# NVIDIA/cuopt

Hardware: AMD Instinct MI355X
Metric: pdlp_iterations_per_sec (higher is better)
Workload: dtype f64; 1 GPU; c3: synthetic random sparse LP S(m=1000000,n=1000000,k=10,seed=2), nnz=10000000, longest row 10, CSR fp64/int32, Stable2 preset, tolerances 0 (fixed iteration budget); rows=1000000, cols=1000000, nnz=10000000, parallelism=single GPU

## Files before the change

### cuopt_amd/capi.py

```python
import ctypes as C
import os

import numpy as np

_HERE = os.path.dirname(os.path.abspath(__file__))
LIB_PATH = os.environ.get("CUOPT_AMD_LIB") or os.path.join(_HERE, "lib", "libcuopt.so")

if not os.path.exists(LIB_PATH):
    raise ImportError(
        "cuopt_amd: %s is missing -- build it with `make -C cuopt_amd/csrc` (or "
        "`python -c 'import __graft_entry__ as g; g.build()'`). There is no CPU fallback." % LIB_PATH)

lib = C.CDLL(LIB_PATH, mode=C.RTLD_GLOBAL)

CUOPT_SUCCESS, CUOPT_INVALID_ARGUMENT, CUOPT_MPS_FILE_ERROR, CUOPT_MPS_PARSE_ERROR = 0, 1, 2, 3
CUOPT_VALIDATION_ERROR, CUOPT_OUT_OF_MEMORY, CUOPT_RUNTIME_ERROR = 4, 5, 6
CUOPT_MINIMIZE, CUOPT_MAXIMIZE = 1, -1
STATUS = {0: "NoTermination", 1: "Optimal", 2: "PrimalInfeasible", 3: "DualInfeasible",
          4: "IterationLimit", 5: "TimeLimit", 6: "NumericalError", 7: "PrimalFeasible",
          8: "FeasibleFound", 9: "ConcurrentLimit"}

c_int, c_double, c_void_p, c_char_p = C.c_int32, C.c_double, C.c_void_p, C.c_char_p
P = C.POINTER

# ... 254 lines not shown
if hasattr(lib, "pdlpdev_loop_stats"):
    _proto("pdlpdev_loop_stats", c_int, c_void_p, c_void_p)
    _proto("pdlpdev_run_period", c_int, c_void_p, c_int, c_void_p, c_void_p, c_void_p, c_void_p, c_void_p)
_proto("pdlpdev_save_best", c_int, c_void_p, c_int)
_proto("pdlpdev_trust_region_bounds", c_int, c_void_p, c_int, c_double, c_double, c_double, c_double, c_double, c_double, c_int, c_void_p)
_proto("pdlpdev_eval_infeasibility", c_int, c_void_p, c_int, c_int, c_void_p)
_proto("pdlpdev_get_solution", c_int, c_void_p, c_int, c_void_p, c_void_p, c_void_p)
_proto("pdlpdev_download", C.c_int64, c_void_p, c_int, c_void_p, C.c_int64)
_proto("pdlpdev_upload", C.c_int64, c_void_p, c_int, c_void_p, C.c_int64)
_proto("pdlpdev_spmv", c_int, c_void_p, c_int, c_void_p, c_void_p)
_proto("pdlpdev_time_kernel", c_int, c_void_p, c_int, c_int, P(c_double))
_proto("pdlpdev_synchronize", c_int, c_void_p)
_proto("pdlpdev_device_bytes", C.c_int64, c_void_p)
_proto("cuoptamd_dual_simplex", c_int, c_void_p, c_double, c_int, c_void_p, c_void_p, c_void_p, c_void_p, c_void_p, c_void_p, c_void_p)
_proto("cuoptamd_dual_simplex_from", c_int, c_void_p, c_void_p, c_void_p, c_double, c_int, c_void_p, c_void_p, c_void_p, c_void_p, c_void_p, c_void_p, c_void_p)
_proto("pdlpdev_shard_dataflow", c_int, c_void_p)
_proto("pdlpdev_shard_transport", c_int, c_void_p)
_proto("pdlpdev_shard_wire_bytes", c_int, c_void_p, c_void_p)
_proto("pdlpdev_dense_info", c_int, c_void_p, c_void_p)
_proto("pdlpdev_layout_info", c_int, c_void_p, c_void_p)
_proto("pdlpdev_comm_abort", c_int, c_void_p)
if hasattr(lib, "pdlpdev_shard_slice"):
    _proto("pdlpdev_shard_slice", c_int, c_void_p, P(c_int), P(c_int))
    _proto("pdlpdev_owner_layout_info", c_int, c_void_p, c_void_p)
_proto("pdlpdev_analyze", c_int, P(c_void_p), c_int, c_int, c_int, c_void_p, c_void_p, c_void_p, c_int)
_proto("pdlpdev_analysis_info", c_int, c_void_p, c_void_p)
_proto("pdlpdev_analysis_maps", c_int, c_void_p, c_void_p, c_void_p)
_proto("pdlpdev_analysis_download", c_int, c_void_p, c_int, c_void_p, c_void_p, c_void_p)
_proto("pdlpdev_create_from_analysis", c_int, P(c_void_p), c_void_p, c_void_p, c_void_p, c_void_p, c_void_p, c_void_p)
_proto("pdlpdev_analysis_destroy", None, c_void_p)
_proto("pdlpdev_debug_sort_pairs", c_int, c_int, C.c_int64, c_void_p, c_void_p, c_int, c_void_p, c_void_p)
_proto("pdlpdev_debug_scan", c_int, c_int, C.c_int64, c_void_p, c_void_p)
_proto("pdlpdev_debug_layout_checksums", c_int, c_void_p, c_void_p)
_proto("cuoptamd_solver_clone", c_int, c_void_p, c_void_p, c_void_p, c_void_p, c_void_p, c_void_p, P(c_void_p))
_proto("cuoptamd_batch_create", c_int, c_void_p, c_int, P(c_void_p))
_proto("cuoptamd_batch_advance", c_int, c_void_p, c_int, c_void_p)
_proto("cuoptamd_batch_destroy", None, c_void_p)
_proto("cuoptamd_batch_reset", c_int, c_void_p, c_void_p, c_void_p, c_void_p, c_void_p)
_proto("cuoptamd_batch_get_solutions", c_int, c_void_p, c_void_p, c_void_p, c_void_p)
_proto("cuoptamd_batch_branch", c_int, c_void_p, c_void_p, c_void_p, c_void_p)
_proto("cuoptamd_batch_solution_views", c_int, c_void_p, c_void_p, c_void_p, c_void_p)
_proto("cuoptamd_batch_device", c_void_p, c_void_p)
_proto("cuoptamd_batch_stats", c_int, c_void_p, c_void_p)
_proto("cuoptamd_batch_solve_last_path", C.c_char_p)
_proto("pdlpdev_small_batch_create", c_int, P(c_void_p), P(c_void_p), c_int)
_proto("pdlpdev_small_batch_destroy", None, c_void_p)
_proto("pdlpdev_create_share_stream", None, c_void_p)
_proto("pdlpdev_debug_ipc_export", c_int, c_int, c_int, c_void_p, P(c_void_p))
_proto("pdlpdev_debug_ipc_store", c_int, c_int, c_void_p, c_int, c_double)
_proto("pdlpdev_debug_ipc_wait", c_int, c_int, c_void_p, c_int, c_double)
_proto("pdlpdev_resident_size", c_int, c_int, c_int, C.c_int64)
if hasattr(lib, "pdlpdev_resident_tier"):
    _proto("pdlpdev_resident_tier", c_int, c_int, c_int, C.c_int64)
_proto("pdlpdev_batch_time_kernels", c_int, c_void_p, c_int, c_void_p)
_proto("pdlpdev_synthetic_lp", c_int, c_int, c_int, c_int, c_int, C.c_uint64, *([c_void_p] * 8))

if hasattr(lib, "pdlpdev_set_halpern"):
    _proto("pdlpdev_create_no_resident", None, c_int)
    _proto("pdlpdev_set_halpern", c_int, c_void_p, c_int)
    _proto("pdlpdev_spectral_norm", c_int, c_void_p, c_double, c_int, P(c_double), P(c_int))
    _proto("pdlpdev_halpern_restart", c_int, c_void_p, c_double, c_void_p, P(Ctl))
    _proto("pdlpdev_get_halpern", c_int, c_void_p, P(Halpern))
if hasattr(lib, "cuoptamd_solver_get_ray"):
    _proto("cuoptamd_solver_get_ray", c_int, c_void_p, c_void_p, c_void_p)
    _proto("pdlpdev_set_halpern_rays", c_int, c_void_p, c_int)
    _proto("pdlpdev_halpern_eval_infeasibility", c_int, c_void_p, c_int, c_void_p)
# ... 822 lines not shown
        def side(k):
            d = dict(layout=names[int(out[k])], panels=bool(out[k] == 1), workgroups=int(out[k + 1]))
            if out[k] == 3:
                d["lds_gather_saving_pct"] = int(out[k + 2])
            elif out[k] == 4:
                d["padding_pct"] = int(out[k + 2])
            else:
                d["slabs"] = int(out[k + 2])
                if out[k] == 1:
                    d["row_sums"] = "by_nonzero" if out[6 + k // 3] else "by_row"
            return d
        return dict(A=side(0), At=side(3), resident=bool(out[0] == 2))

    def shard_slice(self):
        a, b = c_int(), c_int()
        self._ck(lib.pdlpdev_shard_slice(self.handle, C.byref(a), C.byref(b)))
        return a.value, b.value

    def owner_layout(self):
        out = np.zeros(3, np.int32)
        self._ck(lib.pdlpdev_owner_layout_info(self.handle, _ptr(out)))
        return dict(layout={0: "stream", 1: "panel", 3: "jag", 4: "pb"}[int(out[0])], workgroups=int(out[1]), detail=int(out[2]))

    def wire_bytes(self):
        out = np.zeros(3, np.int64)
        self._ck(lib.pdlpdev_shard_wire_bytes(self.handle, _ptr(out)))
        return dict(halo=bool(out[0]), bytes=int(out[1]), bytes_allgather=int(out[2]))

    def layout_checksums(self):
        out = np.zeros(16, np.uint64)
        self._ck(lib.pdlpdev_debug_layout_checksums(self.handle, _ptr(out)))
        return out

    def dense_info(self):
        out = np.zeros(3, np.int64)
        self._ck(lib.pdlpdev_dense_info(self.handle, _ptr(out)))
        return dict(on=bool(out[0]), segments=int(out[1]), entries=int(out[2]))

    def time_kernel(self, kernel, reps=20):
        ms = c_double()
        self._ck(lib.pdlpdev_time_kernel(self.handle, KERNEL[kernel], int(reps), C.byref(ms)))
        return ms.value

    def close(self):
        if self.owner and self.handle:
            lib.pdlpdev_destroy(self.handle)
        self.handle = None

    def __del__(self):
        try:
            self.close()
        except Exception:
            pass
```

### cuopt_amd/csrc/kernels_layout_build.hip

```cpp
#include <hip/hip_runtime.h>

#include "pdlp_setup.hpp"
#include "setup_primitives.hpp"

namespace {

__global__ void __launch_bounds__(kT) k_panel_count(const int32_t* __restrict__ row0, const int32_t* __restrict__ off,
                                                    const int32_t* __restrict__ idx, int S, int32_t slab_w, int64_t own_from,
                                                    int32_t* __restrict__ count )
{
  __shared__ int c[16];
  if (threadIdx.x < 16) c[threadIdx.x] = 0;
  __syncthreads();
  const int w = blockIdx.x;
  const int32_t a = row0[w], b = row0[w + 1];
  for (int32_t i = a + threadIdx.x; i < b; i += kT) {
    const int32_t k0 = off[i], k1 = off[i + 1];
    if ((int64_t)(k1 - k0) > own_from) continue;
    int s_cur = -1, run = 0;
    for (int32_t k = k0; k < k1; ++k) {
      const int s2 = idx[k] / slab_w;
      if (s2 != s_cur) {
        if (run) atomicAdd(&c[s_cur], run);
        s_cur = s2, run = 0;
// ... 26 lines not shown
  }
  __syncthreads();
  for (int s2 = 0; s2 < S; ++s2) {
    int carry = 0;
    for (int r0 = 0; r0 < stride; r0 += 512) {
      const int r = r0 + threadIdx.x;
      const int v = r < nr ? (int)cnt[s2 * stride + r] : 0;
      int total   = 0;
      const int pre = block_exclusive_scan<512>(v, scratch, &total);
      if (r < stride) cnt[s2 * stride + r] = (unsigned short)(carry + pre);
      carry += total;
    }
  }
  __syncthreads();
  if (!SEG)
    for (int s2 = 0; s2 < S; ++s2) {
      uint16_t* dst = rowptr + rp_base[(size_t)w * S + s2];
      for (int r = threadIdx.x; r < stride; r += 512) dst[r] = cnt[s2 * stride + r];
    }
  __syncthreads();
  for (int32_t r = threadIdx.x; r < nr; r += 512) {
    const int32_t k0 = off[a + r], k1 = off[a + r + 1];
    if ((int64_t)(k1 - k0) > own_from) continue;
    for (int32_t k = k0; k < k1; ++k) {
      const int32_t c = idx[k];
      const int s2    = c / slab_w;
      const int32_t q = tile_ptr[(size_t)w * S + s2] + (int32_t)(cnt[s2 * stride + r]++);
      perm[q] = k;
      col[q]  = SEG ? (int32_t)(((uint32_t)r << kSegColBits) | (uint32_t)(c - s2 * slab_w)) : c;
    }
  }
}


}

int build_panels_device(pdlpdev_ctx* c, pdlpdev_ctx::Panels* dst, int32_t rows, int32_t cols, const int32_t* h_off,
                        const int32_t* d_off, const int32_t* d_idx, const double* d_val, int64_t slab_bytes, bool force)
{
  PanelHost h;
  std::vector<char> is_own;
  int64_t own_nnz = 0, own_from = 0;
  const bool timing = getenv("CUOPT_AMD_TIMING") != nullptr;
  auto t_last = std::chrono::steady_clock::now();
  auto plap = [&](const char* what) {
    if (!timing) return;
    const auto now = std::chrono::steady_clock::now();
    fprintf(stderr, "[cuopt_amd setup]     panels: %-18s %6.2f ms\n", what, 1e3 * std::chrono::duration<double>(now - t_last).count());
    t_last = now;
  };
  if (!panel_plan(&h, rows, cols, h_off, slab_bytes, force, nullptr, &is_own, &own_nnz, &own_from)) return 0;
  plap("plan");
  const int W = h.W, S = h.S;
  const int64_t nnz = h_off[rows];
  h.nnz = (size_t)(nnz - own_nnz), h.rowptr_size = h.seg ? 0 : (size_t)S * ((size_t)rows + W);
  int32_t *row0 = nullptr, *tile_ptr = nullptr, *col = nullptr, *count = nullptr;
  uint16_t* rowptr = nullptr;
  int64_t* rp_base = nullptr;
  TRY(upload_i32(c, &row0, h.row0.data(), h.row0.size()));
  TRY(dev_alloc(c, &count, (size_t)W * S + 1));
  k_panel_count<<<W, kT, 0, c->stream>>>(row0, d_off, d_idx, S, h.slab_w, own_from, count);
  std::vector<int32_t> hc((size_t)W * S);
  HIP_TRY(hipMemcpyAsync(hc.data(), count, hc.size() * sizeof(int32_t), hipMemcpyDeviceToHost, c->stream));
  HIP_TRY(hipStreamSynchronize(c->stream));
  plap("count");
  h.tile_ptr.resize((size_t)W * S + 1);
// ... 12 lines not shown
      for (int s2 = 0; s2 < S; ++s2) h.rp_base[(size_t)w * S + s2] = rp + (int64_t)s2 * (nr + 1);
    }
  TRY(upload_i32(c, &tile_ptr, h.tile_ptr.data(), h.tile_ptr.size()));
  {
    auto pad = [](size_t b) { return (b + 255) & ~(size_t)255; };
    const size_t b_col = pad((h.nnz + 8) * sizeof(int32_t)), b_rp = pad((h.rowptr_size + 8) * sizeof(uint16_t)), b_val = pad((h.nnz + 8) * sizeof(double));
    char* block = nullptr;
    HIP_TRY(hipMalloc((void**)&block, 2 * b_col + b_rp + b_val));
    c->allocs.push_back(block);
    c->bytes += (int64_t)(2 * b_col + b_rp + b_val);
    dst->val  = (double*)block;
    col       = (int32_t*)(block + b_val);
    dst->perm = (int32_t*)(block + b_val + b_col);
    rowptr    = (uint16_t*)(block + b_val + 2 * b_col);
  }
  TRY(dev_alloc(c, &rp_base, h.rp_base.size()));
  HIP_TRY(hipMemcpyAsync(rp_base, h.rp_base.data(), h.rp_base.size() * sizeof(int64_t), hipMemcpyHostToDevice, c->stream));
  plap("alloc");
  {
    const size_t lds = (size_t)S * (kPanelMaxRows + 1) * sizeof(unsigned short);
    static std::mutex mu;
    static std::vector<int> done;
    {
      std::lock_guard<std::mutex> lock(mu);
      if (std::find(done.begin(), done.end(), c->device) == done.end()) {
        HIP_TRY(hipFuncSetAttribute((const void*)k_panel_place<false>, hipFuncAttributeMaxDynamicSharedMemorySize, 16 * (kPanelMaxRows + 1) * 2));
        HIP_TRY(hipFuncSetAttribute((const void*)k_panel_place<true>, hipFuncAttributeMaxDynamicSharedMemorySize, 16 * (kPanelMaxRows + 1) * 2));
        done.push_back(c->device);
      }
    }
    if (h.seg) k_panel_place<true><<<W, 512, lds, c->stream>>>(row0, d_off, d_idx, S, h.slab_w, own_from, tile_ptr, rp_base, rowptr, dst->perm, col);
    else k_panel_place<false><<<W, 512, lds, c->stream>>>(row0, d_off, d_idx, S, h.slab_w, own_from, tile_ptr, rp_base, rowptr, dst->perm, col);
    HIP_TRY(hipGetLastError());
  }
  HIP_TRY(hipStreamSynchronize(c->stream));
  plap("place");
  dst->v = PanelView{h.W, h.S, h.any_long ? 1 : 0, row0, tile_ptr, rowptr, rp_base, col, dst->val};
  dst->v.seg = h.seg ? 1 : 0, dst->v.slab_w = h.slab_w;
  dst->nent  = (int64_t)h.nnz;
  if (!h.own_row.empty()) {
    int32_t *own_row = nullptr, *own_ptr = nullptr;
    TRY(upload_i32(c, &own_row, h.own_row.data(), h.own_row.size()));
    TRY(upload_i32(c, &own_ptr, h.own_ptr.data(), h.own_ptr.size()));
    HIP_TRY(hipStreamSynchronize(c->stream));
    dst->v.NP = h.W, dst->v.W = h.W + (int)h.own_row.size();
    dst->v.own_row = own_row, dst->v.own_ptr = own_ptr;
    dst->v.csr_off = d_off, dst->v.csr_idx = d_idx, dst->v.csr_val = d_val;
  }
  dst->on = true;
  return 0;
}

namespace {
constexpr int kPbBinT  = 1024;
constexpr int kPbSortN = 16384;
static_assert(kPbCap <= kPbSortN && kPbMaxRows <= 1024, "a bin's entries / rows fit the LDS sorts");

__global__ void __launch_bounds__(kT) k_max_row_len(int32_t rows, const int32_t* __restrict__ off, int* __restrict__ out)
{
  int best = 0;
  for (int64_t r = (int64_t)blockIdx.x * kT + threadIdx.x; r < rows; r += (int64_t)gridDim.x * kT) best = max(best, off[r + 1] - off[r]);
  for (int d = 1; d < 64; d <<= 1) best = max(best, __shfl_xor(best, d, 64));
  if ((threadIdx.x & 63) == 0 && best > 0) atomicMax(out, best);
}

constexpr int kPbItems = (kPbCap + kPbBinT - 1) / kPbBinT;
template <int MODE>
__global__ void __launch_bounds__(kPbBinT)
k_pb_bin(const int32_t* __restrict__ row0, const int32_t* __restrict__ off, const int32_t* __restrict__ idx, int panel_shift, int gshift, int S, int B,
         int32_t* __restrict__ bin_size, int* __restrict__ maxpad, uint16_t* __restrict__ cnt, const int32_t* __restrict__ pstart,
         const int32_t* __restrict__ bin_e0, int32_t* __restrict__ perm, uint16_t* __restrict__ lidx, int32_t* __restrict__ piece_dst,
// ... 1099 lines not shown
```

### cuopt_amd/csrc/kernels_panel.hip

```cpp
#include <hip/hip_runtime.h>

#include "pdlp_kernel_decls.hpp"
#include "pdlp_layouts.hpp"
#include "pdlp_setup.hpp"
#include "spmv_panel.hpp"

template <bool SEG>
__global__ void __launch_bounds__(kPanelThreads)
k_panel_a_dual(PanelView P, const pdlpdev_ctl* __restrict__ ctl, const double* __restrict__ xbar,
               double* __restrict__ y0, double* __restrict__ y1, const double* __restrict__ lo,
               const double* __restrict__ hi, double* __restrict__ sumy, double* __restrict__ part, double* __restrict__ ycopy,
               const p2pdev::Push* __restrict__ push)
{
  if (!loop_active(ctl)) return;
  DualEpilogue e = DualEpilogue::make(ctl, y0, y1, lo, hi, sumy, ycopy, push);
  const bool masked = !SEG && P.zmask != nullptr && (P.zforce != 0 || ctl->zskip != 0);
  if (masked && blockIdx.x == 0 && threadIdx.x == 0)
    __hip_atomic_fetch_add(const_cast<unsigned long long*>(P.zmask) + 2 * ((size_t)(P.zcols + 127) / 128), 1ull, __ATOMIC_RELAXED, __HIP_MEMORY_SCOPE_AGENT);
  panel_block_zs<SEG>(P, xbar, e, part, masked);
  if (push) p2pdev::count_exchange(push);
}

template <bool SEG>
__global__ void __launch_bounds__(kPanelThreads)
// ... 177 lines not shown
                const std::vector<int32_t>* dense_first_seg, std::vector<char>* is_own_out, int64_t* own_nnz_out, int64_t* own_from_out)
{
  PanelHost& P = *out;
  const int64_t nnz = rows > 0 ? off[rows] : 0;
  if (rows <= 0 || cols <= 0 || nnz <= 0) return false;
  if (!force && (int64_t)cols * 8 <= 2 * (int64_t)1048576) return false;
  int S = (int)(((int64_t)cols * 8 + slab_bytes - 1) / slab_bytes);
  S     = std::max(1, std::min(S, 16));
  const int32_t slab_w = (cols + S - 1) / S;
  const int64_t cap = std::max<int64_t>(2048, cuopt_amd::tune_int("panel_nnz", 60000));
  int64_t long_nnz = 0;
  int32_t max_len  = 0;
  {
    constexpr int kParts = 16;
    int64_t part_long[kParts] = {0};
    int32_t part_max[kParts]  = {0};
    cuopt_amd::parallel_tasks(kParts, [&](int t) {
      const int32_t a = (int32_t)((int64_t)rows * t / kParts), b = (int32_t)((int64_t)rows * (t + 1) / kParts);
      int64_t ln = 0;
      int32_t mx = 0;
      for (int32_t i = a; i < b; ++i) {
        const int32_t len = off[i + 1] - off[i];
        if (len > kLongRow) ln += len;
        mx = std::max(mx, len);
      }
      part_long[t] = ln, part_max[t] = mx;
    }, (int64_t)rows * 8);
    for (int t = 0; t < kParts; ++t) long_nnz += part_long[t], max_len = std::max(max_len, part_max[t]);
  }
  {
    const long long want = cuopt_amd::tune_int("panel_seg", -1);
    P.seg = want == 1 || (want != 0 && long_nnz * 50 > nnz);
    if (slab_w > (1 << kSegColBits)) P.seg = false;
  }
  const int64_t own_from = P.seg ? std::max<int64_t>(kPanelOwnRow, std::min<int64_t>(cap, (nnz + 511) / 512)) : kPanelOwnRow;
  std::vector<char>& is_own = *is_own_out;
  is_own.assign((size_t)rows, 0);
  int64_t own_nnz = 0;
  const bool any_own = max_len > own_from || dense_first_seg != nullptr;
  if (any_own)
    for (int32_t i = 0; i < rows; ++i)
      if (off[i + 1] - off[i] > own_from || (dense_first_seg && (*dense_first_seg)[i] >= 0))
        is_own[i] = 1, P.own_row.push_back(i), own_nnz += off[i + 1] - off[i];
  auto cut = [&](int64_t tgt) {
    P.row0.assign(1, 0);
    int32_t start = 0;
    if (!any_own) {
      while (start < rows) {
        const int32_t last = (int32_t)std::min<int64_t>(rows, (int64_t)start + kPanelMaxRows);
        const int64_t lim  = (int64_t)off[start] + tgt;
        int32_t end = (int32_t)(std::upper_bound(off + start, off + last + 1, lim, [](int64_t v, int32_t o) { return v < (int64_t)o; }) - off) - 1;
        if (end < last && off[end] == off[start]) ++end;
        end = std::max(end, start + 1);
        P.row0.push_back(end);
        start = end;
      }
      return;
    }
    while (start < rows) {
      int32_t end = start;
      int64_t cnt = 0;
      while (end < rows && end - start < kPanelMaxRows) {
        const int64_t len = is_own[end] ? 0 : off[end + 1] - off[end];
        if (cnt > 0 && cnt + len > tgt) break;
        cnt += len;
        ++end;
// ... 61 lines not shown
        if (is_own[i]) continue;
        for (int32_t t = off[i]; t < off[i + 1]; ++t) {
          const int s2    = idx[t] / slab_w;
          const int32_t q = cursor[s2]++;
          P.perm[q] = t, P.col[q] = (int32_t)(((uint32_t)(i - a) << kSegColBits) | (uint32_t)(idx[t] - s2 * slab_w));
        }
      }
    }, nnz);
    P.ok = true;
    return P;
  }
  P.rowptr.reset(P.rowptr_size);
  P.rp_base.resize((size_t)W * S);
  cuopt_amd::parallel_tasks(W, [&](int w) {
    const int32_t a = P.row0[w], b = P.row0[w + 1], nr = b - a;
    const int64_t rp = (int64_t)S * ((int64_t)a + w);
    std::vector<int32_t> cursor(S);
    for (int s2 = 0; s2 < S; ++s2) {
      cursor[s2]                    = P.tile_ptr[(size_t)w * S + s2];
      P.rp_base[(size_t)w * S + s2] = rp + (int64_t)s2 * (nr + 1);
    }
    for (int32_t i = a; i < b; ++i) {
      for (int s2 = 0; s2 < S; ++s2)
        P.rowptr[(size_t)(P.rp_base[(size_t)w * S + s2] + (i - a))] = (uint16_t)(cursor[s2] - P.tile_ptr[(size_t)w * S + s2]);
      if (is_own[i]) continue;
      for (int32_t t = off[i]; t < off[i + 1]; ++t) {
        const int s2 = idx[t] / slab_w;
        const int32_t q = cursor[s2]++;
        P.perm[q] = t, P.col[q] = idx[t];
      }
    }
    for (int s2 = 0; s2 < S; ++s2)
      P.rowptr[(size_t)(P.rp_base[(size_t)w * S + s2] + nr)] = (uint16_t)(cursor[s2] - P.tile_ptr[(size_t)w * S + s2]);
  }, nnz);
  P.ok = true;
  return P;
}

int upload_panels(pdlpdev_ctx* c, pdlpdev_ctx::Panels* dst, const PanelHost& h, const int32_t* d_off, const int32_t* d_idx,
                         const double* d_val)
{
  if (!h.ok) return 0;
  int32_t *row0 = nullptr, *tile_ptr = nullptr, *col = nullptr;
  uint16_t* rowptr = nullptr;
  int64_t* rp_base = nullptr;
  TRY(upload_i32(c, &row0, h.row0.data(), h.row0.size()));
  TRY(upload_i32(c, &tile_ptr, h.tile_ptr.data(), h.tile_ptr.size()));
  TRY(upload_i32(c, &col, h.col.get(), h.nnz));
  TRY(upload_i32(c, &dst->perm, h.perm.get(), h.nnz));
  TRY(dev_alloc(c, &rowptr, h.rowptr_size));
  HIP_TRY(hipMemcpyAsync(rowptr, h.rowptr.get(), h.rowptr_size * sizeof(uint16_t), hipMemcpyHostToDevice, c->stream));
  TRY(dev_alloc(c, &rp_base, h.rp_base.size()));
  HIP_TRY(hipMemcpyAsync(rp_base, h.rp_base.data(), h.rp_base.size() * sizeof(int64_t), hipMemcpyHostToDevice, c->stream));
  TRY(dev_alloc(c, &dst->val, h.nnz));
  HIP_TRY(hipStreamSynchronize(c->stream));
  dst->v  = PanelView{h.W, h.S, h.any_long ? 1 : 0, row0, tile_ptr, rowptr, rp_base, col, dst->val};
  dst->v.seg = h.seg ? 1 : 0, dst->v.slab_w = h.slab_w;
  dst->nent = (int64_t)h.nnz;
  if (!h.own_row.empty()) {
    int32_t *own_row = nullptr, *own_ptr = nullptr;
    TRY(upload_i32(c, &own_row, h.own_row.data(), h.own_row.size()));
    TRY(upload_i32(c, &own_ptr, h.own_ptr.data(), h.own_ptr.size()));
    HIP_TRY(hipStreamSynchronize(c->stream));
    dst->v.NP = h.W, dst->v.W = h.W + (int)h.own_row.size();
    dst->v.own_row = own_row, dst->v.own_ptr = own_ptr;
    dst->v.csr_off = d_off, dst->v.csr_idx = d_idx, dst->v.csr_val = d_val;
  }
  dst->on = true;
  return 0;
}

int pick_layout(pdlpdev_ctx* c, pdlpdev_ctx::MatrixSide* side, const double* vec, double* out)
{
  pdlpdev_ctx::Panels* pn = &side->pan;
  if (!pn->on) return 0;
  hipEvent_t e0, e1;
  HIP_TRY(hipEventCreate(&e0));
  HIP_TRY(hipEventCreate(&e1));
  float ms_stream = 1e30f, ms_panel = 1e30f;
  for (int round = 0; round < 2; ++round)
    for (int which = 0; which < 2; ++which) {
      for (int rep = 0; rep < 4; ++rep) {
        if (rep == 1) HIP_TRY(hipEventRecord(e0, c->stream));
        if (which == 0)
          k_spmv_plain<<<stream_grid(side->nb), kBlock, 0, c->stream>>>(side->nb, side->rb, side->hot.off, side->hot.idx, side->hot.val, vec, out, (const double*)nullptr);
        else
          (pn->v.seg ? k_panel_plain<true> : k_panel_plain<false>)<<<pn->v.W, kPanelThreads, 0, c->stream>>>(pn->v, vec, out);
      }
      HIP_TRY(hipEventRecord(e1, c->stream));
      HIP_TRY(hipEventSynchronize(e1));
// ... 15 lines not shown
```

### cuopt_amd/csrc/pdlp_device.hip

```cpp
#include "pdlp_ctx.hpp"
#include "pdlp_layouts.hpp"
#include "pdlp_setup.hpp"
#include "halpern_decision.hpp"


__global__ void __launch_bounds__(kBlock) k_fill(int64_t n, double* __restrict__ d, double v)
{
  for (int64_t i = blockIdx.x * (int64_t)kBlock + threadIdx.x; i < n; i += (int64_t)gridDim.x * kBlock)
    d[i] = v;
}
__global__ void __launch_bounds__(kBlock) k_scale_vectors(int n, int m, double* __restrict__ c,
                                                          double* __restrict__ lb,
                                                          double* __restrict__ ub,
                                                          const double* __restrict__ dc,
                                                          double* __restrict__ lo,
                                                          double* __restrict__ hi,
                                                          const double* __restrict__ dr)
{
  const int tot = n > m ? n : m;
  for (int i = blockIdx.x * kBlock + threadIdx.x; i < tot; i += gridDim.x * kBlock) {
    if (i < n) {
      c[i]  = c[i] * dc[i];
      lb[i] = lb[i] / dc[i];
      ub[i] = ub[i] / dc[i];
// ... 1583 lines not shown
  return 0;
}
int64_t pdlpdev_device_bytes(pdlpdev_ctx* ctx) { return ctx->bytes; }
int pdlpdev_shard_dataflow(pdlpdev_ctx* ctx) { return !ctx->comm ? 0 : ctx->owner ? 3 : ctx->rsag ? 2 : 1; }
int pdlpdev_shard_transport(pdlpdev_ctx* ctx) { return ctx->p2p.on ? 1 : 0; }
int pdlpdev_shard_wire_bytes(pdlpdev_ctx* ctx, int64_t out[3])
{
  out[0] = ctx->halo.on ? 1 : 0, out[1] = ctx->halo.on ? ctx->halo.bytes : ctx->halo.bytes_allgather, out[2] = ctx->halo.bytes_allgather;
  return 0;
}
int pdlpdev_dense_info(pdlpdev_ctx* ctx, int64_t out[3])
{
  out[0] = ctx->dense.on ? 1 : 0, out[1] = ctx->dense.nseg, out[2] = ctx->dense.nent;
  return 0;
}
int pdlpdev_layout_info(pdlpdev_ctx* ctx, int32_t out[8])
{
  ctx->A.info(out), ctx->At.info(out + 3);
  out[6] = ctx->A.pan.on && ctx->A.pan.v.seg, out[7] = ctx->At.pan.on && ctx->At.pan.v.seg;
  if (ctx->small_resident) out[0] = out[3] = 2;
  return 0;
}

static uint64_t checksum_device(pdlpdev_ctx* ctx, const void* dev, size_t bytes)
{
  if (!dev || bytes == 0) return 0;
  std::vector<unsigned char> h(bytes);
  if (hipMemcpy(h.data(), dev, bytes, hipMemcpyDeviceToHost) != hipSuccess) return ~0ull;
  uint64_t f = 1469598103934665603ull;
  for (unsigned char b : h) f = (f ^ b) * 1099511628211ull;
  (void)ctx;
  return f;
}
int pdlpdev_debug_layout_checksums(pdlpdev_ctx* ctx, uint64_t out[16])
{
  HIP_TRY(hipSetDevice(ctx->device));
  HIP_TRY(hipStreamSynchronize(ctx->stream));
  for (int i = 0; i < 16; ++i) out[i] = 0;
  const size_t nnz = (size_t)ctx->nnz;
  out[0] = checksum_device(ctx, ctx->At.full.off, ((size_t)ctx->n + 1) * 4);
  out[1] = checksum_device(ctx, ctx->At.full.idx, nnz * 4);
  out[2] = checksum_device(ctx, ctx->At.full.val, nnz * 8);
  auto panels = [&](const pdlpdev_ctx::Panels& P, int32_t rows, uint64_t* o) {
    if (!P.on) return;
    const int NP = P.v.NP ? P.v.NP : P.v.W;
    o[0] = checksum_device(ctx, P.v.row0, ((size_t)NP + 1) * 4);
    o[1] = checksum_device(ctx, P.v.tile_ptr, ((size_t)NP * P.v.S + 1) * 4);
    o[2] = P.v.seg ? 0 : checksum_device(ctx, P.v.rowptr, (size_t)P.v.S * ((size_t)rows + NP) * 2);
    o[3] = checksum_device(ctx, P.v.col, (size_t)P.nent * 4);
    o[4] = checksum_device(ctx, P.perm, (size_t)P.nent * 4);
  };
  panels(ctx->A.pan, ctx->m, out + 3);
  panels(ctx->At.pan, ctx->n, out + 8);
  auto gather_free = [&](const pdlpdev_ctx::Pb& P, int64_t side_nnz, uint64_t* o) {
    if (!P.on) return;
    const PbView& v = P.v;
    o[0] = checksum_device(ctx, P.perm, (size_t)P.np * 4);
    o[1] = checksum_device(ctx, v.lidx, (size_t)P.np * 2);
    o[2] = checksum_device(ctx, v.piece_dst, (size_t)(P.np >> v.gshift) * 4);
    o[4] = checksum_device(ctx, v.wg_e0, ((size_t)v.nwg + 1) * 4) ^ (checksum_device(ctx, v.wg_panel, (size_t)v.nwg * 4) * 3) ^
           (checksum_device(ctx, v.bin_row0, ((size_t)v.B + 1) * 4) * 5) ^ (checksum_device(ctx, v.bin_e0, ((size_t)v.B + 1) * 4) * 7) ^
           (uint64_t)v.S * 17 ^ (uint64_t)v.gshift * 19 ^ (uint64_t)v.panel_shift * 23 ^ (uint64_t)P.p_threads * 29 ^ (uint64_t)v.wide * 31;
    if (v.wide) {
      o[3] = checksum_device(ctx, v.rib, (size_t)P.np * 2) ^ (checksum_device(ctx, v.step_lv, (size_t)(P.np >> 10)) * 3) ^ (uint64_t)v.nser * 37;
      if (v.nser) {
        int32_t ser_nnz = 0;
// ... 35 lines not shown
```

### cuopt_amd/csrc/pdlp_kernels.hpp

```cpp
#pragma once
#include <hip/hip_runtime.h>
#include <stdint.h>


#include "cuopt_amd/pdlp_device.h"

namespace pdlp {

typedef double vec4d __attribute__((ext_vector_type(4)));
typedef int vec4i __attribute__((ext_vector_type(4)));

constexpr int kBlock    = 256;
constexpr int kNnzTile  = 2048;
constexpr int kNnzBlock = kNnzTile - 4;
constexpr int kLongRow  = 128;
constexpr int kMaxRowsPerBlock = 1024;

template <int XOR_MASK>
__device__ __forceinline__ double swizzle_xor(double v)
{
  static_assert(XOR_MASK >= 1 && XOR_MASK <= 16, "ds_swizzle works inside 32 lanes");
  constexpr int pattern = (XOR_MASK << 10) | 0x1F;
  int lo = __double2loint(v), hi = __double2hiint(v);
  lo = __builtin_amdgcn_ds_swizzle(lo, pattern);
// ... 97 lines not shown
constexpr int kPeriodGuard = 0x100;
__device__ __forceinline__ bool period_guard_skips(const pdlpdev_ctl* ctl, int& arg)
{
  const bool guarded = (arg & kPeriodGuard) != 0;
  arg &= ~kPeriodGuard;
  return guarded && !period_reached(ctl);
}

__device__ __forceinline__ int xcd_remap(int b, int nb)
{
  const int per = (nb + 7) >> 3;
  const int v   = (b & 7) * per + (b >> 3);
  return v;
}



constexpr int kPanelThreads = 512;
constexpr int kPanelChunk   = 4096;
constexpr int kPanelMaxRows = 3584;
constexpr int kPanelWaves   = kPanelThreads / 64;

struct PanelView {
  int W, S;
  int any_long;
  const int32_t* __restrict__ row0;
  const int32_t* __restrict__ tile_ptr;
  const uint16_t* __restrict__ rowptr;
  const int64_t* __restrict__ rp_base;
  const int32_t* __restrict__ col;
  const double* __restrict__ val;
  const double* __restrict__ dense_add = nullptr;
  int seg = 0, slab_w = 0;
  int NP = 0;
  const int32_t* __restrict__ own_row = nullptr;
  const int32_t* __restrict__ own_ptr = nullptr;
  const int32_t* __restrict__ csr_off = nullptr;
  const int32_t* __restrict__ csr_idx = nullptr;
  const double* __restrict__ csr_val  = nullptr;
  const int32_t* __restrict__ dn_own_seg   = nullptr;
  const int32_t* __restrict__ dn_pan_ptr   = nullptr;
  const int32_t* __restrict__ dn_pan_seg   = nullptr;
  const int32_t* __restrict__ dn_seg_row   = nullptr;
  const int32_t* __restrict__ dn_seg_c0    = nullptr;
  const int32_t* __restrict__ dn_seg_len   = nullptr;
  const int32_t* __restrict__ dn_seg_ptr   = nullptr;
  const double* __restrict__ dn_val        = nullptr;
  const unsigned long long* __restrict__ zmask = nullptr;
  int zcols = 0, zforce = 0;
};
constexpr int kZsQuads        = 1152;
constexpr int kPanelOwnRow = 4096;
constexpr int kPanelDenseSegs = 32;
constexpr long long kPanelNotMine = 0x7FF8C0DEC0DEC0DELL;

constexpr int kPanelPer     = kPanelChunk / kPanelThreads;
constexpr int kPanelRowsPer = (kPanelMaxRows + kPanelThreads - 1) / kPanelThreads;
constexpr int kSegColBits = 20;
constexpr unsigned kSegColMask = (1u << kSegColBits) - 1u;

constexpr int kJagMaxGroup = 256;
constexpr int kJagBatchRows = 16384;
#ifndef CUOPT_AMD_JAG_U
#define CUOPT_AMD_JAG_U 8
#endif
constexpr int kJagU        = CUOPT_AMD_JAG_U;
constexpr int jag_window(int waves) { return waves == 16 ? 16384 : 8192; }
constexpr size_t jag_lds_bytes(int waves) { return sizeof(double) * (size_t)(jag_window(waves) + waves * kJagMaxGroup); }
constexpr long long kJagNotMine = 0x7FF8C0DEC0DEC0DELL;

struct JagView {
  int rows, waves, ngroups, nblk, nlong;
  const int32_t* __restrict__ row0;
  const int32_t* __restrict__ tile_e;
  const int32_t* __restrict__ tile_sr;
  const uint32_t* __restrict__ sr;
  const uint16_t* __restrict__ slot;
  const double* __restrict__ val;
  const int32_t* __restrict__ win;
  const int32_t* __restrict__ set_ptr;
  const int32_t* __restrict__ set_col;
  const int32_t* __restrict__ lr_ptr;
  const int32_t* __restrict__ lr_row;
  const int32_t* __restrict__ off;
  const int32_t* __restrict__ idx;
  const double* __restrict__ csr_val;
  const double* __restrict__ dense_add = nullptr;
};


constexpr int kPbThreads = 512;
constexpr int kPbCap     = 9088;
// ... 166 lines not shown
```

### cuopt_amd/csrc/pdlp_layouts.hpp

```cpp
#pragma once
#include "pdlp_ctx.hpp"

struct PanelHost {
  bool ok = false, any_long = false;
  bool seg = false;
  int32_t slab_w = 0;
  int W = 0, S = 0;
  std::vector<int32_t> own_row, own_ptr;
  std::vector<int32_t> row0, tile_ptr;
  std::vector<int64_t> rp_base;
  cuopt_amd::PoolArray<int32_t> perm, col;
  cuopt_amd::PoolArray<uint16_t> rowptr;
  size_t nnz = 0, rowptr_size = 0;
};

constexpr int64_t kPanelWorkingSetBytes = 4 * (int64_t)1048576;

struct LayoutPolicy {
  enum Mode { kAuto, kStream, kPanel, kJag, kPb, kTimed } mode = kAuto;
  int64_t slab_bytes = 0;
  int64_t ws_limit   = 0;
  bool pb_device = true, jag_device = true;
  bool try_jag() const { return mode == kAuto || mode == kJag || mode == kTimed; }
  bool want_pb(int32_t cols) const { return mode == kPb || (mode == kAuto && (int64_t)cols * 8 > 16 * slab_bytes); }
};
int layout_policy(LayoutPolicy* p);

struct JagHost {
  bool ok = false;
  int rows = 0, waves = 8, ngroups = 0, nblk = 0;
  std::vector<int32_t> row0, tile_e, tile_sr, win, set_ptr, set_col, lr_ptr, lr_row;
  cuopt_amd::PoolArray<uint32_t> sr;
  cuopt_amd::PoolArray<uint16_t> slot;
  cuopt_amd::PoolArray<int32_t> perm;
  size_t nsr = 0, nent = 0;
  double saving = 0.0;
};

// ... 91 lines not shown
```

### cuopt_amd/csrc/spmv_panel.hpp

```cpp
#pragma once
#include <type_traits>

#include "pdlp_kernels.hpp"

namespace pdlp {

struct PanelChunk {
  int s, c0, c1, t0;
  bool valid;
};
template <int R>
__device__ __forceinline__ void panel_load(const PanelView& P, double (&va)[kPanelPer], int (&ja)[kPanelPer], int c0, int c1)
{
#pragma unroll
  for (int u = 0; u < R; ++u) {
    int k = c0 + threadIdx.x + u * kPanelThreads;
    if (u == R - 1) k = k < c1 ? k : c1 - 1;
    va[u] = __builtin_nontemporal_load(P.val + k);
    ja[u] = __builtin_nontemporal_load(P.col + k);
  }
}
template <int R>
__device__ __forceinline__ void panel_products(const double* __restrict__ vec, double* prod, const double (&va)[kPanelPer],
                                               const int (&ja)[kPanelPer], int len)
{
  double x[R];
#pragma unroll
  for (int u = 0; u < R; ++u) x[u] = vec[ja[u]];
#pragma unroll
  for (int u = 0; u < R; ++u) {
    const int i = threadIdx.x + u * kPanelThreads;
    if (u < R - 1 || i < len) prod[i] = va[u] * x[u];
  }
}
template <int R>
__device__ __forceinline__ void panel_products_zs(const double* __restrict__ vec, double* prod, const double (&va)[kPanelPer],
                                                  const int (&ja)[kPanelPer], int len, const unsigned* zbits, int zbase)
{
  unsigned w[R];
#pragma unroll
  for (int u = 0; u < R; ++u) {
    const int wi = (ja[u] >> 5) - zbase;
    w[u]         = wi < kZsQuads * 4 ? zbits[wi] : ~0u;
  }
  double x[R];
#pragma unroll
  for (int u = 0; u < R; ++u) {
    x[u] = 0.0;
    if ((w[u] >> (ja[u] & 31)) & 1u) x[u] = vec[ja[u]];
  }
#pragma unroll
  for (int u = 0; u < R; ++u) {
    const int i = threadIdx.x + u * kPanelThreads;
    if (u < R - 1 || i < len) prod[i] = va[u] * x[u];
  }
}
constexpr int kZsPer = (kZsQuads + kPanelThreads - 1) / kPanelThreads;
__device__ __forceinline__ int panel_zs_first_quad(const PanelView& P, int s) { return (int)(((long long)s * P.slab_w) >> 7); }
__device__ __forceinline__ void panel_zs_load(const PanelView& P, int s, uint4 (&st)[kZsPer])
{
  const long long c1 = (long long)(s + 1) * P.slab_w;
  const int last     = (int)(c1 < P.zcols ? c1 : P.zcols) - 1;
  const int q0       = panel_zs_first_quad(P, s);
  int nq             = (last >> 7) - q0 + 1;
  nq                 = nq < kZsQuads ? nq : kZsQuads;
  const uint4* __restrict__ src = reinterpret_cast<const uint4*>(P.zmask) + q0;
#pragma unroll
  for (int k = 0; k < kZsPer; ++k) {
    const int q = threadIdx.x + k * kPanelThreads;
    st[k]       = uint4{0u, 0u, 0u, 0u};
    if (q < nq) st[k] = src[q];
  }
}
__device__ __forceinline__ void panel_zs_store(uint4* zq, const uint4 (&st)[kZsPer])
{
#pragma unroll
  for (int k = 0; k < kZsPer; ++k) {
    const int q = threadIdx.x + k * kPanelThreads;
    if (q < kZsQuads) zq[q] = st[k];
  }
}
#define PANEL_DISPATCH(rounds, CALL) \
  switch (rounds) {                   \
    case 1: CALL(1); break;           \
    case 2: CALL(2); break;           \
    case 3: CALL(3); break;           \
    case 4: CALL(4); break;           \
// ... 246 lines not shown
    panel_own_row(P, vec, epi, partials, w, NP, prod);
    return;
  }
  __shared__ PanelDenseSegs dseg;
  const int r0 = P.row0[w], nr = P.row0[w + 1] - r0;
  panel_dense_prepare(P, w, vec, &dseg);
  if (threadIdx.x <= P.S) tile_s[threadIdx.x] = P.tile_ptr[w * P.S + threadIdx.x];
  if (threadIdx.x < P.S) base_s[threadIdx.x] = P.rp_base[w * P.S + threadIdx.x];
  for (int r = threadIdx.x; r < nr; r += kPanelThreads) psum[r] = 0.0;
  __syncthreads();
  if (P.own_ptr)
    for (int q = P.own_ptr[w] + (int)threadIdx.x; q < P.own_ptr[w + 1]; q += kPanelThreads) psum[P.own_row[q] - r0] = __longlong_as_double(kPanelNotMine);
  auto advance = [&](PanelChunk c) -> PanelChunk {
    if (c.valid && c.c1 < tile_s[c.s + 1]) {
      c.c0 = c.c1;
      c.c1 = c.c0 + kPanelChunk < tile_s[c.s + 1] ? c.c0 + kPanelChunk : tile_s[c.s + 1];
      return c;
    }
    int s = c.s + 1;
    while (s < P.S && tile_s[s + 1] == tile_s[s]) ++s;
    c.valid = s < P.S;
    c.s     = s;
    if (c.valid) {
      c.t0 = c.c0 = tile_s[s];
      c.c1 = c.c0 + kPanelChunk < tile_s[s + 1] ? c.c0 + kPanelChunk : tile_s[s + 1];
    }
    return c;
  };
  double va[kPanelPer];
  int ja[kPanelPer];
  unsigned ext_next[kPanelRowsPer], ext[kPanelRowsPer];
#define PANEL_ROUNDS(c) (((c).c1 - (c).c0 + kPanelThreads - 1) / kPanelThreads)
#define PANEL_CALL_LOAD(R) panel_load<R>(P, va, ja, nxt.c0, nxt.c1)
#define PANEL_CALL_PRODUCTS(R) panel_products<R>(vec, prod, va, ja, cur.c1 - cur.c0)
#define PANEL_CALL_PRODUCTS_ZS(R) panel_products_zs<R>(vec, prod, va, ja, cur.c1 - cur.c0, reinterpret_cast<const unsigned*>(zq), panel_zs_first_quad(P, cur.s) << 2)
#define PANEL_REQUEST(c)                                                         \
  if ((c).valid) {                                                               \
    PANEL_DISPATCH(PANEL_ROUNDS(c), PANEL_CALL_LOAD)                             \
    const uint16_t* __restrict__ rp_ = P.rowptr + base_s[(c).s];                 \
    _Pragma("unroll") for (int q = 0; q < kPanelRowsPer; ++q) {                  \
      int r_      = threadIdx.x + q * kPanelThreads;                             \
      r_          = r_ < nr ? r_ : 0;                                            \
      ext_next[q] = (unsigned)rp_[r_] | ((unsigned)rp_[r_ + 1] << 16);           \
    }                                                                            \
  }
  PanelChunk none{-1, 0, 0, 0, false};
  PanelChunk nxt = advance(none);
  PANEL_REQUEST(nxt)
  PanelChunk cur = nxt;
  if (zon && cur.valid) {
    uint4 st[kZsPer];
    panel_zs_load(P, cur.s, st);
    panel_zs_store(zq, st);
  }
  constexpr bool kEarly = PanelEarlyOps<Epi>::on;
  [[maybe_unused]] typename PanelEarlyOps<Epi>::type pre[kPanelEpiDepth];
  [[maybe_unused]] int lo_last = 0, hi_last = 0;
  while (cur.valid) {
    __syncthreads();
    if (zon) { PANEL_DISPATCH(PANEL_ROUNDS(cur), PANEL_CALL_PRODUCTS_ZS) }
    else { PANEL_DISPATCH(PANEL_ROUNDS(cur), PANEL_CALL_PRODUCTS) }
#pragma unroll
    for (int q = 0; q < kPanelRowsPer; ++q) ext[q] = ext_next[q];
    const int lo = cur.c0 - cur.t0, hi = cur.c1 - cur.t0;
    nxt = advance(cur);
    if constexpr (kEarly)
      if (!nxt.valid) {
        lo_last = lo, hi_last = hi;
// ... 235 lines not shown
```

### include/cuopt_amd/pdlp_device.h

```cpp
#ifndef CUOPT_AMD_PDLP_DEVICE_H
#define CUOPT_AMD_PDLP_DEVICE_H

#include <stdint.h>

#ifdef __cplusplus
extern "C" {
#endif

typedef struct pdlpdev_ctx pdlpdev_ctx;

typedef struct pdlpdev_ctl {
  double step_size;
  double primal_weight;
  double tau;
  double sigma;
  double sum_weights;
  double last_interaction, last_movement, last_dx2, last_dy2;
  int32_t k;
  int32_t cur;
  int32_t pending_avg;
  int32_t steps_taken;
  int32_t attempts;
  int32_t target_steps;
  int32_t error;
// ... 94 lines not shown
void pdlpdev_create_no_resident(int no_resident);
void pdlpdev_create_batch_lanes(int lanes);
void pdlpdev_create_share_stream(pdlpdev_ctx* donor);
int pdlpdev_resident_size(int32_t m, int32_t n, int64_t nnz);
int pdlpdev_resident_tier(int32_t m, int32_t n, int64_t nnz);
int pdlpdev_create_overlapped(pdlpdev_ctx** out, int device, int32_t m, int32_t n, const int32_t* a_offsets,
                              const int32_t* a_indices, const double* a_values, const int32_t* at_offsets,
                              const int32_t* at_indices, const double* at_values,
                              void (*transpose_ready)(void*), void* user, const double* c, const double* lo,
                              const double* hi, const double* lb, const double* ub);
void pdlpdev_destroy(pdlpdev_ctx* ctx);

typedef struct pdlpdev_analysis pdlpdev_analysis;
int pdlpdev_analyze(pdlpdev_analysis** out, int device, int32_t m, int32_t n, const int32_t* a_offsets, const int32_t* a_indices,
                    const double* a_values, int flags);
int pdlpdev_analyze_with_vectors(pdlpdev_analysis** out, int device, int32_t m, int32_t n, const int32_t* a_offsets, const int32_t* a_indices,
                                 const double* a_values, int flags, const double* c, const double* lo, const double* hi, const double* lb,
                                 const double* ub);
int pdlpdev_analysis_info(pdlpdev_analysis* an, int32_t out[10]);
int pdlpdev_analysis_maps(pdlpdev_analysis* an, int32_t* row_new2old, int32_t* col_new2old);
int pdlpdev_analysis_vectors_in_order(pdlpdev_analysis* an);
void pdlpdev_analysis_release_workspace(pdlpdev_analysis* an);
int pdlpdev_analysis_download(pdlpdev_analysis* an, int which, int32_t* offsets, int32_t* indices, double* values);
int pdlpdev_create_from_analysis(pdlpdev_ctx** out, pdlpdev_analysis* an, const double* c, const double* lo, const double* hi,
                                 const double* lb, const double* ub);
void pdlpdev_analysis_destroy(pdlpdev_analysis* an);
int pdlpdev_debug_sort_pairs(int device, int64_t n, const uint32_t* keys, const uint32_t* vals, int bits, uint32_t* keys_out,
                             uint32_t* vals_out);
int pdlpdev_debug_scan(int device, int64_t n, const int32_t* in, int32_t* out);
int pdlpdev_debug_ipc_export(int device, int count, uint8_t handle[64], void** base);
int pdlpdev_debug_ipc_store(int device, const uint8_t handle[64], int count, double seed);
int pdlpdev_debug_ipc_wait(int device, void* base, int count, double seed);
int pdlpdev_debug_layout_checksums(pdlpdev_ctx* ctx, uint64_t out[16]);
int pdlpdev_debug_pb_wide_host(int32_t rows, int32_t cols, const int32_t* off, const int32_t* idx, const double* val, const double* x, double* out,
                               int64_t info[5]);
int pdlpdev_synthetic_lp(int device, int32_t m, int32_t n, int32_t k, uint64_t seed, int32_t* offsets, int32_t* indices, double* values,
                         double* c, double* lo, double* hi, double* x_star, double* y_star);

int pdlpdev_comm_unique_id(uint8_t id[128]);
int pdlpdev_comm_init(pdlpdev_ctx* ctx, int rank, int world, const uint8_t id[128]);

int pdlpdev_softcomm_create(int world, uint8_t id[128]);
int pdlpdev_comm_abort(const uint8_t id[128]);

int pdlpdev_scaling_compute(pdlpdev_ctx* ctx, int do_ruiz, int ruiz_iterations,
                            int do_pock_chambolle, double alpha);
int pdlpdev_scale_problem(pdlpdev_ctx* ctx);
int pdlpdev_init_norms(pdlpdev_ctx* ctx, double out[3]);
int pdlpdev_agree_max(pdlpdev_ctx* ctx, double* value);
int pdlpdev_weight_norms(pdlpdev_ctx* ctx, int unscaled, double out[2]);
int pdlpdev_reset(pdlpdev_ctx* ctx, const double* lb, const double* ub, const double* lo, const double* hi);
int pdlpdev_problem_norms(pdlpdev_ctx* ctx, double* norm_c, double* norm_b);
int pdlpdev_set_step_params(pdlpdev_ctx* ctx, const pdlpdev_step_params* p);
int pdlpdev_set_step(pdlpdev_ctx* ctx, double step_size, double primal_weight);
int pdlpdev_set_k(pdlpdev_ctx* ctx, int32_t k);
int pdlpdev_set_initial(pdlpdev_ctx* ctx, const double* x, const double* y);
int pdlpdev_project_primal(pdlpdev_ctx* ctx);
int pdlpdev_initial_solution_stats(pdlpdev_ctx* ctx, double out[5], const double* x0_unscaled, const double* y0_unscaled);

int pdlpdev_compute_aty(pdlpdev_ctx* ctx);
int pdlpdev_run(pdlpdev_ctx* ctx, int32_t target_steps, pdlpdev_ctl* ctl);
int pdlpdev_get_ctl(pdlpdev_ctx* ctx, pdlpdev_ctl* ctl);
typedef struct pdlpdev_batch pdlpdev_batch;
int pdlpdev_clone_shared(pdlpdev_ctx** out, pdlpdev_ctx* parent);
int pdlpdev_batch_create(pdlpdev_batch** out, pdlpdev_ctx** ctx, int K);
int pdlpdev_batch_run(pdlpdev_batch* batch, const int32_t* targets, pdlpdev_ctl* ctl);
// ... 85 lines not shown
```

Baseline: 6570 iterations/s.

## Sort panel chunk entries by column to improve gather locality in SpMV

Within each panel tile chunk, entries are reordered by column (on host and via a device bitonic sort kernel), with each column word packing the original slot index in its high bits. The SpMV product step decodes the column and scatters the product back to its original LDS slot, so x-vector gathers become more coalesced/cache-friendly. This costs extra decode ALU work, a scattered LDS write, and setup-time sorting; it is enabled by default for non-segmented panels.

New measurement: 6773 iterations/s (median of 6 runs). 3.1% higher.

```diff
diff --git a/cuopt_amd/capi.py b/cuopt_amd/capi.py
--- a/cuopt_amd/capi.py
+++ b/cuopt_amd/capi.py
@@ -310,6 +310,8 @@
 _proto("pdlpdev_debug_sort_pairs", c_int, c_int, C.c_int64, c_void_p, c_void_p, c_int, c_void_p, c_void_p)
 _proto("pdlpdev_debug_scan", c_int, c_int, C.c_int64, c_void_p, c_void_p)
 _proto("pdlpdev_debug_layout_checksums", c_int, c_void_p, c_void_p)
+if hasattr(lib, "pdlpdev_debug_panel_words"):
+    _proto("pdlpdev_debug_panel_words", c_int, c_void_p, c_int, c_void_p, c_void_p, c_void_p)
 _proto("cuoptamd_solver_clone", c_int, c_void_p, c_void_p, c_void_p, c_void_p, c_void_p, c_void_p, P(c_void_p))
 _proto("cuoptamd_batch_create", c_int, c_void_p, c_int, P(c_void_p))
 _proto("cuoptamd_batch_advance", c_int, c_void_p, c_int, c_void_p)
@@ -1198,6 +1200,13 @@
         self._ck(lib.pdlpdev_debug_layout_checksums(self.handle, _ptr(out)))
         return out
 
+    def panel_words(self, side):
+        which, info = dict(A=0, At=1)[side], np.zeros(5, np.int64)
+        self._ck(lib.pdlpdev_debug_panel_words(self.handle, which, _ptr(info), None, None))
+        tile_ptr, col = np.zeros(int(info[0] * info[1]) + 1, np.int32), np.zeros(int(info[2]), np.int32)
+        self._ck(lib.pdlpdev_debug_panel_words(self.handle, which, _ptr(info), _ptr(tile_ptr), _ptr(col)))
+        return dict(panels=int(info[0]), slabs=int(info[1]), sorted=bool(info[3]), slab_w=int(info[4]), tile_ptr=tile_ptr, col=col)
+
     def dense_info(self):
         out = np.zeros(3, np.int64)
         self._ck(lib.pdlpdev_dense_info(self.handle, _ptr(out)))
diff --git a/cuopt_amd/csrc/kernels_layout_build.hip b/cuopt_amd/csrc/kernels_layout_build.hip
--- a/cuopt_amd/csrc/kernels_layout_build.hip
+++ b/cuopt_amd/csrc/kernels_layout_build.hip
@@ -82,6 +82,38 @@
   }
 }
 
+__global__ void __launch_bounds__(512) k_panel_sort(int S, int32_t slab_w, const int32_t* __restrict__ tile_ptr, int32_t* __restrict__ perm,
+                                                    int32_t* __restrict__ col)
+{
+  __shared__ uint32_t key[kPanelChunk];
+  __shared__ int32_t pm[kPanelChunk];
+  const int32_t t1 = tile_ptr[blockIdx.x + 1], base = (int32_t)(blockIdx.x % (unsigned)S) * slab_w;
+  for (int32_t c0 = tile_ptr[blockIdx.x]; c0 < t1; c0 += kPanelChunk) {
+    const int len = t1 - c0 < kPanelChunk ? t1 - c0 : kPanelChunk;
+    int n = 2;
+    while (n < len) n <<= 1;
+    for (int i = threadIdx.x; i < n; i += 512) {
+      key[i] = i < len ? ((uint32_t)(col[c0 + i] - base) << 12) | (uint32_t)i : 0xFFFFFFFFu;
+      if (i < len) pm[i] = perm[c0 + i];
+    }
+    __syncthreads();
+    for (int k = 2; k <= n; k <<= 1)
+      for (int j = k >> 1; j > 0; j >>= 1) {
+        for (int t = threadIdx.x; t < (n >> 1); t += 512) {
+          const int lo = ((t & ~(j - 1)) << 1) | (t & (j - 1)), hi = lo | j;
+          const uint32_t a = key[lo], b = key[hi];
+          if ((a > b) == ((lo & k) == 0)) key[lo] = b, key[hi] = a;
+        }
+        __syncthreads();
+      }
+    for (int i = threadIdx.x; i < len; i += 512) {
+      const uint32_t slot = key[i] & 0xFFFu;
+      col[c0 + i]  = (int32_t)((slot << kSegColBits) | (key[i] >> 12));
+      perm[c0 + i] = pm[slot];
+    }
+    __syncthreads();
+  }
+}
 
 }
 
@@ -160,11 +192,15 @@
     if (h.seg) k_panel_place<true><<<W, 512, lds, c->stream>>>(row0, d_off, d_idx, S, h.slab_w, own_from, tile_ptr, rp_base, rowptr, dst->perm, col);
     else k_panel_place<false><<<W, 512, lds, c->stream>>>(row0, d_off, d_idx, S, h.slab_w, own_from, tile_ptr, rp_base, rowptr, dst->perm, col);
     HIP_TRY(hipGetLastError());
+    if (h.sorted) {
+      k_panel_sort<<<W * S, 512, 0, c->stream>>>(S, h.slab_w, tile_ptr, dst->perm, col);
+      HIP_TRY(hipGetLastError());
+    }
   }
   HIP_TRY(hipStreamSynchronize(c->stream));
   plap("place");
   dst->v = PanelView{h.W, h.S, h.any_long ? 1 : 0, row0, tile_ptr, rowptr, rp_base, col, dst->val};
-  dst->v.seg = h.seg ? 1 : 0, dst->v.slab_w = h.slab_w;
+  dst->v.seg = h.seg ? 1 : 0, dst->v.slab_w = h.slab_w, dst->v.sorted = h.sorted ? 1 : 0;
   dst->nent  = (int64_t)h.nnz;
   if (!h.own_row.empty()) {
     int32_t *own_row = nullptr, *own_ptr = nullptr;
diff --git a/cuopt_amd/csrc/kernels_panel.hip b/cuopt_amd/csrc/kernels_panel.hip
--- a/cuopt_amd/csrc/kernels_panel.hip
+++ b/cuopt_amd/csrc/kernels_panel.hip
@@ -233,6 +233,7 @@
     const long long want = cuopt_amd::tune_int("panel_seg", -1);
     P.seg = want == 1 || (want != 0 && long_nnz * 50 > nnz);
     if (slab_w > (1 << kSegColBits)) P.seg = false;
+    P.sorted = !P.seg && slab_w <= (1 << kSegColBits) && cuopt_amd::tune_int("panel_sort", 1) != 0;
   }
   const int64_t own_from = P.seg ? std::max<int64_t>(kPanelOwnRow, std::min<int64_t>(cap, (nnz + 511) / 512)) : kPanelOwnRow;
   std::vector<char>& is_own = *is_own_out;
@@ -360,6 +361,20 @@
     }
     for (int s2 = 0; s2 < S; ++s2)
       P.rowptr[(size_t)(P.rp_base[(size_t)w * S + s2] + nr)] = (uint16_t)(cursor[s2] - P.tile_ptr[(size_t)w * S + s2]);
+    if (!P.sorted) return;
+    std::vector<uint32_t> key;
+    std::vector<int32_t> pm;
+    for (int s2 = 0; s2 < S; ++s2)
+      for (int32_t c0 = P.tile_ptr[(size_t)w * S + s2], t1 = P.tile_ptr[(size_t)w * S + s2 + 1]; c0 < t1; c0 += kPanelChunk) {
+        const int32_t len = std::min<int32_t>(kPanelChunk, t1 - c0);
+        key.resize((size_t)len), pm.assign(&P.perm[c0], &P.perm[c0] + len);
+        for (int32_t i = 0; i < len; ++i) key[i] = ((uint32_t)(P.col[c0 + i] - s2 * slab_w) << 12) | (uint32_t)i;
+        std::sort(key.begin(), key.end());
+        for (int32_t i = 0; i < len; ++i) {
+          const uint32_t slot = key[i] & 0xFFFu;
+          P.col[c0 + i] = (int32_t)((slot << kSegColBits) | (key[i] >> 12)), P.perm[c0 + i] = pm[slot];
+        }
+      }
   }, nnz);
   P.ok = true;
   return P;
@@ -383,7 +398,7 @@
   TRY(dev_alloc(c, &dst->val, h.nnz));
   HIP_TRY(hipStreamSynchronize(c->stream));
   dst->v  = PanelView{h.W, h.S, h.any_long ? 1 : 0, row0, tile_ptr, rowptr, rp_base, col, dst->val};
-  dst->v.seg = h.seg ? 1 : 0, dst->v.slab_w = h.slab_w;
+  dst->v.seg = h.seg ? 1 : 0, dst->v.slab_w = h.slab_w, dst->v.sorted = h.sorted ? 1 : 0;
   dst->nent = (int64_t)h.nnz;
   if (!h.own_row.empty()) {
     int32_t *own_row = nullptr, *own_ptr = nullptr;
diff --git a/cuopt_amd/csrc/pdlp_device.hip b/cuopt_amd/csrc/pdlp_device.hip
--- a/cuopt_amd/csrc/pdlp_device.hip
+++ b/cuopt_amd/csrc/pdlp_device.hip
@@ -1639,6 +1639,18 @@
   (void)ctx;
   return f;
 }
+int pdlpdev_debug_panel_words(pdlpdev_ctx* ctx, int side, int64_t info[5], int32_t* tile_ptr, int32_t* col)
+{
+  HIP_TRY(hipSetDevice(ctx->device));
+  HIP_TRY(hipStreamSynchronize(ctx->stream));
+  const pdlpdev_ctx::Panels& P = side ? ctx->At.pan : ctx->A.pan;
+  if (!P.on) return fail(-1, "side %d is not in panels", side);
+  const int NP = P.v.NP ? P.v.NP : P.v.W;
+  info[0] = NP, info[1] = P.v.S, info[2] = P.nent, info[3] = P.v.sorted, info[4] = P.v.slab_w;
+  if (tile_ptr) HIP_TRY(hipMemcpy(tile_ptr, P.v.tile_ptr, ((size_t)NP * P.v.S + 1) * 4, hipMemcpyDeviceToHost));
+  if (col) HIP_TRY(hipMemcpy(col, P.v.col, (size_t)P.nent * 4, hipMemcpyDeviceToHost));
+  return 0;
+}
 int pdlpdev_debug_layout_checksums(pdlpdev_ctx* ctx, uint64_t out[16])
 {
   HIP_TRY(hipSetDevice(ctx->device));
diff --git a/cuopt_amd/csrc/pdlp_kernels.hpp b/cuopt_amd/csrc/pdlp_kernels.hpp
--- a/cuopt_amd/csrc/pdlp_kernels.hpp
+++ b/cuopt_amd/csrc/pdlp_kernels.hpp
@@ -153,6 +153,7 @@
   const double* __restrict__ val;
   const double* __restrict__ dense_add = nullptr;
   int seg = 0, slab_w = 0;
+  int sorted = 0;
   int NP = 0;
   const int32_t* __restrict__ own_row = nullptr;
   const int32_t* __restrict__ own_ptr = nullptr;
@@ -179,6 +180,7 @@
 constexpr int kPanelRowsPer = (kPanelMaxRows + kPanelThreads - 1) / kPanelThreads;
 constexpr int kSegColBits = 20;
 constexpr unsigned kSegColMask = (1u << kSegColBits) - 1u;
+static_assert(kPanelChunk <= 1 << 12, "a sorted chunk's slot takes the 12 bits beside the column");
 
 constexpr int kJagMaxGroup = 256;
 constexpr int kJagBatchRows = 16384;
diff --git a/cuopt_amd/csrc/pdlp_layouts.hpp b/cuopt_amd/csrc/pdlp_layouts.hpp
--- a/cuopt_amd/csrc/pdlp_layouts.hpp
+++ b/cuopt_amd/csrc/pdlp_layouts.hpp
@@ -4,6 +4,7 @@
 struct PanelHost {
   bool ok = false, any_long = false;
   bool seg = false;
+  bool sorted = false;
   int32_t slab_w = 0;
   int W = 0, S = 0;
   std::vector<int32_t> own_row, own_ptr;
diff --git a/cuopt_amd/csrc/spmv_panel.hpp b/cuopt_amd/csrc/spmv_panel.hpp
--- a/cuopt_amd/csrc/spmv_panel.hpp
+++ b/cuopt_amd/csrc/spmv_panel.hpp
@@ -20,39 +20,52 @@
     ja[u] = __builtin_nontemporal_load(P.col + k);
   }
 }
+__device__ __forceinline__ void panel_decode(int word, int i, bool sorted, int slab_base, int& col, int& slot)
+{
+  col  = sorted ? slab_base + (int)((unsigned)word & kSegColMask) : word;
+  slot = sorted ? (int)((unsigned)word >> kSegColBits) : i;
+}
 template <int R>
 __device__ __forceinline__ void panel_products(const double* __restrict__ vec, double* prod, const double (&va)[kPanelPer],
-                                               const int (&ja)[kPanelPer], int len)
+                                               const int (&ja)[kPanelPer], int len, bool sorted, int slab_base)
 {
   double x[R];
-#pragma unroll
-  for (int u = 0; u < R; ++u) x[u] = vec[ja[u]];
+  int slot[R];
+#pragma unroll
+  for (int u = 0; u < R; ++u) {
+    int c;
+    panel_decode(ja[u], threadIdx.x + u * kPanelThreads, sorted, slab_base, c, slot[u]);
+    x[u] = vec[c];
+  }
 #pragma unroll
   for (int u = 0; u < R; ++u) {
     const int i = threadIdx.x + u * kPanelThreads;
-    if (u < R - 1 || i < len) prod[i] = va[u] * x[u];
+    if (u < R - 1 || i < len) prod[slot[u]] = va[u] * x[u];
   }
 }
 template <int R>
 __device__ __forceinline__ void panel_products_zs(const double* __restrict__ vec, double* prod, const double (&va)[kPanelPer],
-                                                  const int (&ja)[kPanelPer], int len, const unsigned* zbits, int zbase)
+                                                  const int (&ja)[kPanelPer], int len, const unsigned* zbits, int zbase, bool sorted,
+                                                  int slab_base)
 {
   unsigned w[R];
-#pragma unroll
-  for (int u = 0; u < R; ++u) {
-    const int wi = (ja[u] >> 5) - zbase;
+  int c[R], slot[R];
+#pragma unroll
+  for (int u = 0; u < R; ++u) {
+    panel_decode(ja[u], threadIdx.x + u * kPanelThreads, sorted, slab_base, c[u], slot[u]);
+    const int wi = (c[u] >> 5) - zbase;
     w[u]         = wi < kZsQuads * 4 ? zbits[wi] : ~0u;
   }
   double x[R];
 #pragma unroll
   for (int u = 0; u < R; ++u) {
     x[u] = 0.0;
-    if ((w[u] >> (ja[u] & 31)) & 1u) x[u] = vec[ja[u]];
+    if ((w[u] >> (c[u] & 31)) & 1u) x[u] = vec[c[u]];
   }
 #pragma unroll
   for (int u = 0; u < R; ++u) {
     const int i = threadIdx.x + u * kPanelThreads;
-    if (u < R - 1 || i < len) prod[i] = va[u] * x[u];
+    if (u < R - 1 || i < len) prod[slot[u]] = va[u] * x[u];
   }
 }
 constexpr int kZsPer = (kZsQuads + kPanelThreads - 1) / kPanelThreads;
@@ -365,8 +378,8 @@
   unsigned ext_next[kPanelRowsPer], ext[kPanelRowsPer];
 #define PANEL_ROUNDS(c) (((c).c1 - (c).c0 + kPanelThreads - 1) / kPanelThreads)
 #define PANEL_CALL_LOAD(R) panel_load<R>(P, va, ja, nxt.c0, nxt.c1)
-#define PANEL_CALL_PRODUCTS(R) panel_products<R>(vec, prod, va, ja, cur.c1 - cur.c0)
-#define PANEL_CALL_PRODUCTS_ZS(R) panel_products_zs<R>(vec, prod, va, ja, cur.c1 - cur.c0, reinterpret_cast<const unsigned*>(zq), panel_zs_first_quad(P, cur.s) << 2)
+#define PANEL_CALL_PRODUCTS(R) panel_products<R>(vec, prod, va, ja, cur.c1 - cur.c0, P.sorted != 0, cur.s * P.slab_w)
+#define PANEL_CALL_PRODUCTS_ZS(R) panel_products_zs<R>(vec, prod, va, ja, cur.c1 - cur.c0, reinterpret_cast<const unsigned*>(zq), panel_zs_first_quad(P, cur.s) << 2, P.sorted != 0, cur.s * P.slab_w)
 #define PANEL_REQUEST(c)                                                         \
   if ((c).valid) {                                                               \
     PANEL_DISPATCH(PANEL_ROUNDS(c), PANEL_CALL_LOAD)                             \
diff --git a/include/cuopt_amd/pdlp_device.h b/include/cuopt_amd/pdlp_device.h
--- a/include/cuopt_amd/pdlp_device.h
+++ b/include/cuopt_amd/pdlp_device.h
@@ -150,6 +150,7 @@
 int pdlpdev_debug_ipc_store(int device, const uint8_t handle[64], int count, double seed);
 int pdlpdev_debug_ipc_wait(int device, void* base, int count, double seed);
 int pdlpdev_debug_layout_checksums(pdlpdev_ctx* ctx, uint64_t out[16]);
+int pdlpdev_debug_panel_words(pdlpdev_ctx* ctx, int side, int64_t info[5], int32_t* tile_ptr, int32_t* col);
 int pdlpdev_debug_pb_wide_host(int32_t rows, int32_t cols, const int32_t* off, const int32_t* idx, const double* val, const double* x, double* out,
                                int64_t info[5]);
 int pdlpdev_synthetic_lp(int device, int32_t m, int32_t n, int32_t k, uint64_t seed, int32_t* offsets, int32_t* indices, double* values,
```
